# zafarrafii/Zaf-Python

Hardware: AMD Instinct MI355X
Metric: audio Msamples/sec (STFT win=2048 hop=1024) (higher is better)
Workload: dtype f32

## Files before the change

### zaf-python_amd/csrc/zafx_stft.hip

```cpp
#include <algorithm>
#include <type_traits>

#include "zafx_fft.hpp"
#include "zafx_units.hpp"
#include "zafx_internal.hpp"

namespace zafx {

template <int SPEC>
__device__ __forceinline__ float2* spec_base(float2* out, long long off) {
    if constexpr (SPEC >= 2) return reinterpret_cast<float2*>(reinterpret_cast<float*>(out) + off);
    else return out + off;
}
template <int SPEC, bool STREAM = false>
__device__ __forceinline__ void put_bin(float2* o, long long idx, float2 v) {
    if constexpr (SPEC >= 2) {
        const float pw = v.x * v.x + v.y * v.y;
        reinterpret_cast<float*>(o)[idx] = SPEC == 2 ? __builtin_amdgcn_sqrtf(pw) : pw;
    } else if constexpr (STREAM) {
        store_stream(o + idx, v);
    } else {
        o[idx] = v;
    }
}

template <int LOG2N, int LOG2E, int FPB>
struct StftCfg {
    using C = FftCfg<LOG2N, LOG2E>;
    static constexpr int NT = FPB * C::P;
    static constexpr bool TW_LDS = (size_t)(FPB * C::PITCH + C::TW) * 8 <= (size_t)kMaxLdsBytes;
    static constexpr size_t SMEM = (size_t)(FPB * C::PITCH + (TW_LDS ? C::TW : 0)) * 8;
};

template <int LOG2N, int LOG2E, int FPB, int LAYOUT, int SPEC>
__global__ __launch_bounds__(FPB * fft_threads(LOG2N, LOG2E)) void k_stft(
    const float* __restrict__ x, const float* __restrict__ win, const float2* __restrict__ twp,
    const float2* __restrict__ tws, float2* __restrict__ out, long long n_samples, int hop, int T, int TP, int tiles) {
    using C = FftCfg<LOG2N, LOG2E>;
    using S = StftCfg<LOG2N, LOG2E, FPB>;
    constexpr int N = C::N, P = C::P, E = C::E, W = 2 * N, NT = S::NT, ROWS = SPEC ? N + 1 : W;
    extern __shared__ __attribute__((aligned(16))) unsigned char smem_raw[];
    float2* frames = reinterpret_cast<float2*>(smem_raw);
    const float2* tw = twp;
    const int tid = threadIdx.x;
    if constexpr (S::TW_LDS) {
        float2* tw_l = frames + FPB * C::PITCH;
        for (int i = tid; i < C::TW; i += NT) tw_l[i] = twp[i];
        tw = tw_l;
        __syncthreads();
    }
    const int slot = tid / P, p = tid % P;
    const int bid = ZAFX_XCD_ORDER ? xcd_order((int)blockIdx.x, (int)gridDim.x) : (int)blockIdx.x;
    const int clip = bid / tiles, tile = bid % tiles;
    const int t0 = tile * FPB;
    const int t = t0 + slot;
    float2* buf = frames + slot * C::PITCH;

    float2 v[E];
    {
        const float* xc = x + (long long)clip * n_samples;
        const long long s0 = (long long)t * hop - N;
        const float2* w2 = reinterpret_cast<const float2*>(win);
        if (t < T && s0 >= 0 && s0 + W <= n_samples && reinterpret_cast<uintptr_t>(xc + s0) % 8 == 0) {
            const float2* x2 = reinterpret_cast<const float2*>(xc + s0);
#pragma unroll
            for (int i = 0; i < E; ++i) {
                const int n = p + i * P;
                const float2 xv = x2[n], wv = w2[n];
                v[i] = make_float2(xv.x * wv.x, xv.y * wv.y);
            }
        } else {
#pragma unroll
            for (int i = 0; i < E; ++i) {
                const int n = p + i * P;
                const long long s = s0 + 2 * n;
                const float2 wv = w2[n];
                const float a = (t < T && s >= 0 && s < n_samples) ? xc[s] : 0.f;
                const float b = (t < T && s + 1 >= 0 && s + 1 < n_samples) ? xc[s + 1] : 0.f;
                v[i] = make_float2(a * wv.x, b * wv.y);
            }
        }
    }
    fft_frame<LOG2N, LOG2E>(v, buf, p, tw);

    if constexpr (LAYOUT == ZAFX_LAYOUT_TF) {
        if (t >= T) return;
        float2* o = spec_base<SPEC>(out, ((long long)clip * T + t) * ROWS);
#pragma unroll
        for (int i = 0; i < E / 2; ++i) {
            const int k = p + i * P;
            if (k == 0) {
                const float2 z0 = buf[0], zc = buf[phys(N / 2)];
                put_bin<SPEC>(o, 0, make_float2(z0.x + z0.y, 0.f));
                put_bin<SPEC>(o, N, make_float2(z0.x - z0.y, 0.f));
                put_bin<SPEC>(o, N / 2, cconj(zc));
                if (SPEC == 0) put_bin<SPEC>(o, N + N / 2, zc);
            } else {
                float2 xk, xn;
                split_pair(buf[phys(k)], buf[phys(N - k)], tws[k], xk, xn);
                put_bin<SPEC>(o, k, xk);
                put_bin<SPEC>(o, N - k, xn);
                if (SPEC == 0) {
                    put_bin<SPEC>(o, W - k, cconj(xk));
                    put_bin<SPEC>(o, N + k, cconj(xn));
                }
            }
        }
    } else {
        if constexpr (NT > 64) __syncthreads();
        const int tt = tid % FPB, kq = tid / FPB;
        if (t0 + tt >= T) return;
        const float2* fb = frames + tt * C::PITCH;
        float2* o = spec_base<SPEC>(out, (long long)clip * ROWS * TP + (t0 + tt));
        for (int k = kq; k < N / 2; k += P) {
            if (k == 0) {
                const float2 z0 = fb[0], zc = fb[phys(N / 2)];
                put_bin<SPEC>(o, 0, make_float2(z0.x + z0.y, 0.f));
                put_bin<SPEC>(o, (long long)N * TP, make_float2(z0.x - z0.y, 0.f));
                put_bin<SPEC>(o, (long long)(N / 2) * TP, cconj(zc));
                if (SPEC == 0) put_bin<SPEC>(o, (long long)(N + N / 2) * TP, zc);
            } else {
                float2 xk, xn;
                split_pair(fb[phys(k)], fb[phys(N - k)], tws[k], xk, xn);
                put_bin<SPEC>(o, (long long)k * TP, xk);
                put_bin<SPEC>(o, (long long)(N - k) * TP, xn);
                if (SPEC == 0) {
                    put_bin<SPEC>(o, (long long)(W - k) * TP, cconj(xk));
                    put_bin<SPEC>(o, (long long)(N + k) * TP, cconj(xn));
                }
            }
        }
    }
}

ZAFX_PROF_ARRAY(g_prof_stft)
ZAFX_PROF_TAIL_PTR(g_stft_tail)
constexpr int kFatWaves = 8;
constexpr int kFatFrames = 16;

template <int LOG2N, int LOG2E, int FPB_ = kFatFrames>
struct FatCfg {
    using C = FftCfg<LOG2N, LOG2E>;
    static_assert(C::P == 64 || C::P == 32, "a frame is owned by one wavefront, or by half of one (32 points per thread)");
    static constexpr int N = C::N;
    static constexpr int FPB = FPB_;
    static constexpr bool WIN_LDS = FPB_ == kFatFrames;
    static constexpr int PITCH = ((N + (N >> C::PS) + 31) / 32) * 32 + 32 / FPB_;
    static constexpr int NT = kFatWaves * 64;
    static constexpr int FPW = FPB_ * C::P / NT;
    static constexpr size_t SMEM = (size_t)(FPB_ * PITCH + C::TW + (WIN_LDS ? N : 0) + N / 2 + 1) * 8;
};

template <int PCM>
struct PcmPoint {
    using T = std::conditional_t<PCM == 1, float, float2>;
    static __device__ __forceinline__ float2 get(T v) {
        if constexpr (PCM == 1) {
            const int d = __builtin_bit_cast(int, v);
            return make_float2((float)(short)(d & 0xffff), (float)(d >> 16));
        } else if constexpr (PCM == 2) {
            const int a = __builtin_bit_cast(int, v.x), b = __builtin_bit_cast(int, v.y);
            return make_float2((float)((int)(short)(a & 0xffff) + (a >> 16)), (float)((int)(short)(b & 0xffff) + (b >> 16)));
        } else {
            return v;
        }
    }
    static constexpr float scale() { return PCM == 1 ? 1.f / 32768.f : PCM == 2 ? 1.f / 65536.f : 1.f; }
};

#ifndef ZAFX_STFT_FAT_OPAQUE
#define ZAFX_STFT_FAT_OPAQUE(log2n, spec) ((log2n) == 8 || ((log2n) == 9 && (spec) <= 1))
#endif
template <int LOG2N, int LOG2E, bool ALIGNED, int SPEC, int FPB_ = kFatFrames, int PCM = 0, bool RAGGED = false, bool DYN = false>
__global__ __launch_bounds__(kFatWaves * 64) void k_stft_ft16(
    const float* __restrict__ x, const float* __restrict__ win, const float2* __restrict__ twp,
    const float2* __restrict__ tws, float2* __restrict__ out, SamplesArg<RAGGED> n_samples, int hop, int T, int TP, int tiles,
    TilesArg<DYN> tiles_arg) {
    static_assert(!RAGGED || (FPB_ == kFatFrames && (PCM == 0 || LOG2N == 10)), "ragged batches: 16-frame tiles; int16 samples at W = 2048");
    static_assert(!DYN || FPB_ == kFatFrames, "claimed tiles: 16-frame tiles");
    const int& total_tiles = tiles_total<DYN>(tiles_arg);
#define CLIP_N rg_pick<RAGGED>(rc.n_samples, n_samples)
#define CLIP_T rg_pick<RAGGED>(rc.T, T)
#define CLIP_TP rg_pick<RAGGED>(rc.TP, TP)
    using C = FftCfg<LOG2N, LOG2E>;
    using F = FatCfg<LOG2N, LOG2E, FPB_>;
    constexpr int N = C::N, P = C::P, E = C::E, W = 2 * N, NT = F::NT, FPB = F::FPB, FPW = F::FPW, PITCH = F::PITCH;
    static_assert(FPW >= 1, "every group of P lanes transforms at least one frame per tile");
    constexpr int ROWS = SPEC ? N + 1 : W;
    extern __shared__ __attribute__((aligned(16))) unsigned char smem_raw[];
    float2* frames = reinterpret_cast<float2*>(smem_raw);
    float2* tw_l = frames + FPB * PITCH;
    float2* win_s = tw_l + C::TW;
    float2* tws_l = win_s + (F::WIN_LDS ? N : 0);
    const float2* win_l = F::WIN_LDS ? win_s : reinterpret_cast<const float2*>(win);
    const int tid = threadIdx.x;
    [[maybe_unused]] int* const slot = reinterpret_cast<int*>(tws_l + N / 2 + 1);
    [[maybe_unused]] const int home = (int)blockIdx.x & (kClaimQueues - 1);
    [[maybe_unused]] int cq = home, ticket = 0;
    [[maybe_unused]] bool live = false;
    [[maybe_unused]] auto draw = [&](int q) { return atomicAdd(tiles_claim<DYN>(tiles_arg) + q * kClaimStride, 1); };
    if constexpr (DYN) {
        if (tid == 0) {
            const int c0 = claim_finish(cq, home, total_tiles, draw(cq), draw);
            const int c1 = c0 >= 0 ? claim_finish(cq, home, total_tiles, draw(cq), draw) : -1;
            slot[2] = c0;
            slot[1] = c1;
            live = c1 >= 0;
        }
    }
    for (int i = tid; i < C::TW; i += NT) tw_l[i] = twp[i];
    static_assert(PCM == 0 || F::WIN_LDS, "int16 input: the staged window carries the scale");
    using PP = PcmPoint<PCM>;
    if constexpr (F::WIN_LDS)
        for (int i = tid; i < N; i += NT) {
            const float2 wv = reinterpret_cast<const float2*>(win)[i];
            win_s[i] = make_float2(wv.x * PP::scale(), wv.y * PP::scale());
        }
    for (int i = tid; i <= N / 2; i += NT) tws_l[i] = tws[i];
    __syncthreads();
    const int wave = tid / P, p_lane = tid % P, p = p_lane;
    const int tt = tid % FPB, kq = tid / FPB;
    const float2* fb = frames + tt * PITCH;
    const bool lines_whole = (RAGGED || TP % 16 == 0) && reinterpret_cast<uintptr_t>(out) % 128 == 0;

    typename PP::T xr[FPW][E];
    [[maybe_unused]] const bool xcd = ZAFX_XCD_ORDER && gridDim.x % 8 == 0;
    auto prefetch = [&](int tlv) {
        if (DYN ? tlv < 0 : tlv >= total_tiles) return;
        const int tl = DYN ? tlv : xcd ? xcd_order(tlv, total_tiles) : tlv;
        int p = p_lane;
        if constexpr (E >= 32 || ZAFX_STFT_FAT_OPAQUE(LOG2N, SPEC)) asm volatile("" : "+v"(p));
        [[maybe_unused]] RgClip rc;
        if constexpr (RAGGED) rc = rg_clip(n_samples, tiles, tl);
        const int clip = RAGGED ? 0 : tl / tiles, tile = RAGGED ? tl - rc.first_tile : tl % tiles;
        const float* xc = x + (RAGGED ? rc.in_off : (long long)clip * CLIP_N);
        const long long first = (long long)tile * FPB * hop - N;
        const long long last = first + (long long)(FPB - 1) * hop + W;
        if constexpr (PCM == 1) {
            const short* xs = reinterpret_cast<const short*>(x) + (RAGGED ? rc.in_off : (long long)clip * CLIP_N);
            if (ALIGNED && first >= 0 && last <= CLIP_N && tile * FPB + FPB <= CLIP_T) {
                const short* src = xs + first + (long long)(wave * FPW) * hop + 2 * p;
#pragma unroll
                for (int f = 0; f < FPW; ++f) {
#pragma unroll
                    for (int i = 0; i < E; ++i) xr[f][i] = *reinterpret_cast<const float*>(src + (long long)f * hop + 2 * i * P);
                }
            } else {
#pragma unroll
                for (int f = 0; f < FPW; ++f) {
                    const int t = tile * FPB + wave * FPW + f;
                    const long long s0 = (long long)t * hop - N;
#pragma unroll
                    for (int i = 0; i < E; ++i) {
                        const long long s = s0 + 2 * (p + i * P);
                        const unsigned lo = (t < CLIP_T && s >= 0 && s < CLIP_N) ? (unsigned short)xs[s] : 0u;
                        const unsigned hi = (t < CLIP_T && s + 1 >= 0 && s + 1 < CLIP_N) ? (unsigned short)xs[s + 1] : 0u;
                        xr[f][i] = __builtin_bit_cast(float, lo | hi << 16);
                    }
                }
            }
        } else if (ALIGNED && first >= 0 && last <= CLIP_N && tile * FPB + FPB <= CLIP_T) {
            const float* src = xc + first + (long long)(wave * FPW) * hop + 2 * p;
#pragma unroll
            for (int f = 0; f < FPW; ++f) {
#pragma unroll
                for (int i = 0; i < E; ++i) xr[f][i] = *reinterpret_cast<const float2*>(src + (long long)f * hop + 2 * i * P);
            }
        } else {
#pragma unroll
            for (int f = 0; f < FPW; ++f) {
                const int t = tile * FPB + wave * FPW + f;
                const long long s0 = (long long)t * hop - N;
#pragma unroll
                for (int i = 0; i < E; ++i) {
                    const long long s = s0 + 2 * (p + i * P);
                    xr[f][i].x = (t < CLIP_T && s >= 0 && s < CLIP_N) ? xc[s] : 0.f;
                    xr[f][i].y = (t < CLIP_T && s + 1 >= 0 && s + 1 < CLIP_N) ? xc[s + 1] : 0.f;
                }
            }
        }
    };
    int tlv = blockIdx.x;
    if constexpr (DYN) tlv = __builtin_amdgcn_readfirstlane(slot[2]);
    [[maybe_unused]] int par = 0;
    prefetch(tlv);
    PROF_INIT(g_prof_stft);
    PROF_TAIL_INIT();
    while (DYN ? tlv >= 0 : tlv < total_tiles) {
        const int tl = DYN ? tlv : xcd ? xcd_order(tlv, total_tiles) : tlv;
        [[maybe_unused]] RgClip rc;
        if constexpr (RAGGED) rc = rg_clip(n_samples, tiles, tl);
        const int clip = RAGGED ? 0 : tl / tiles, tile = RAGGED ? tl - rc.first_tile : tl % tiles;
        const int t0 = tile * FPB;
        PROF_MARK(0);
        int po = p;
        if constexpr (E >= 32 || ZAFX_STFT_FAT_OPAQUE(LOG2N, SPEC)) asm volatile("" : "+v"(po));
#pragma unroll
        for (int f = 0; f < FPW; ++f) {
            float2 v[E];
            if constexpr (DYN) {
                if (f == FPW - 1) {
#pragma unroll
                    for (int i = 0; i < E; ++i) {
                        if constexpr (PCM == 1) asm volatile("" : "+v"(xr[f][i])::"memory");
                        else asm volatile("" : "+v"(xr[f][i].x), "+v"(xr[f][i].y)::"memory");
                    }
                    if (tid == 0 && live) ticket = draw(cq);
                }
            }
#pragma unroll
            for (int i = 0; i < E; ++i) {
                const float2 wv = win_l[po + i * P], xv = PP::get(xr[f][i]);
                v[i] = make_float2(xv.x * wv.x, xv.y * wv.y);
            }
            fft_frame<LOG2N, LOG2E>(v, frames + (wave * FPW + f) * PITCH, po, tw_l);
        }
#ifndef ZAFX_STFT_EARLY
#define ZAFX_STFT_EARLY 1
#endif
        if constexpr (DYN) {
            if (tid == 0) {
                const int c = live ? claim_finish(cq, home, total_tiles, ticket, draw) : -1;
                slot[par] = c;
                live = c >= 0;
            }
        }
        int nxt = tlv + gridDim.x;
        if constexpr (DYN) nxt = __builtin_amdgcn_readfirstlane(slot[par ^ 1]);
        if (ZAFX_STFT_EARLY) prefetch(nxt);
        PROF_MARK(1);
        lds_barrier();
        PROF_MARK(2);
        if (!ZAFX_STFT_EARLY) prefetch(nxt);
        PROF_TAIL_FIRST();
        PROF_MARK(3);
        if (t0 + tt < CLIP_T) {
            float2* o = spec_base<SPEC>(out, (RAGGED ? rc.out_off : (long long)clip * ROWS * TP) + (t0 + tt));
            int kqo = kq;
            if constexpr (E >= 32 || ZAFX_STFT_FAT_OPAQUE(LOG2N, SPEC)) asm volatile("" : "+v"(kqo));
            auto store_tile = [&](auto stream) {
                constexpr bool ST = decltype(stream)::value;
                constexpr int ITER = (N / 2) / (NT / FPB);
#ifndef ZAFX_STFT_ROWROT_EXPR
#define ZAFX_STFT_ROWROT_EXPR (((int)blockIdx.x & 7) * 2 + ((int)blockIdx.x >> 3))
#endif
                static_assert((N / 2) % (NT / FPB) == 0, "the row sweep is a whole number of iterations");
                const int rot = ST ? ZAFX_STFT_ROWROT_EXPR : 0;
                for (int it = 0; it < ITER; ++it) {
                    const int k = kqo + ((it + rot) % ITER) * (NT / FPB);
                    if (k == 0) {
                        const float2 z0 = fb[0], zc = fb[phys_t<C::PS>(N / 2)];
                        put_bin<SPEC, ST>(o, 0, make_float2(z0.x + z0.y, 0.f));
                        put_bin<SPEC, ST>(o, (long long)N * CLIP_TP, make_float2(z0.x - z0.y, 0.f));
                        put_bin<SPEC, ST>(o, (long long)(N / 2) * CLIP_TP, cconj(zc));
                        if (SPEC == 0) put_bin<SPEC, ST>(o, (long long)(N + N / 2) * CLIP_TP, zc);
                    } else {
                        float2 xk, xn;
                        split_pair(fb[phys_t<C::PS>(k)], fb[phys_t<C::PS>(N - k)], tws_l[k], xk, xn);
                        put_bin<SPEC, ST>(o, (long long)k * CLIP_TP, xk);
                        if (SPEC == 0) put_bin<SPEC, ST>(o, (long long)(W - k) * CLIP_TP, cconj(xk));
                        put_bin<SPEC, ST>(o, (long long)(N - k) * CLIP_TP, xn);
                        if (SPEC == 0) put_bin<SPEC, ST>(o, (long long)(N + k) * CLIP_TP, cconj(xn));
                    }
                }
            };
#ifndef ZAFX_STFT_NO_NT
            if (SPEC < 2 && lines_whole && FPB == 16) store_tile(std::true_type{});
            else
#endif
                store_tile(std::false_type{});
        }
        PROF_MARK(4);
        lds_barrier();
        tlv = nxt;
        par ^= 1;
        PROF_TAIL_TILE();
    }
    PROF_TAIL_END(g_stft_tail);
    if constexpr (DYN) {
        if (tid == 0) {
            int* const cnt = tiles_claim<DYN>(tiles_arg);
            if (atomicAdd(cnt + kClaimQueues * kClaimStride, 1) == (int)gridDim.x - 1)
                for (int i = 0; i <= kClaimQueues; ++i) atomicExch(cnt + i * kClaimStride, 0);
        }
    }
}
#undef CLIP_N
#undef CLIP_T
#undef CLIP_TP

template <int LOG2N, int LOG2E, bool ALIGNED, int SPEC, int PCM = 0>
__global__ __launch_bounds__(kFatWaves * 64) void k_stft_ft16c(
    const float* __restrict__ x, const float* __restrict__ win, const float2* __restrict__ twp,
    const float2* __restrict__ tws, float2* __restrict__ out, long long n_samples, int hop, int T, int TP, int tiles,
    int segs, int seg_tiles, int units) {
    static_assert(SPEC < 2, "complex spectra only (the real kinds write 64-byte runs)");
    using C = FftCfg<LOG2N, LOG2E>;
    using F = FatCfg<LOG2N, LOG2E>;
    constexpr int N = C::N, P = C::P, E = C::E, W = 2 * N, NT = F::NT, FPB = kFatFrames, FPW = F::FPW, PITCH = F::PITCH;
    constexpr int ROWS = SPEC ? N + 1 : W;
    constexpr int ITER = (N / 2) / (NT / FPB);
    static_assert((N / 2) % (NT / FPB) == 0 && ITER >= 1, "the row sweep is a whole number of iterations");
    extern __shared__ __attribute__((aligned(16))) unsigned char smem_raw[];
    float2* frames = reinterpret_cast<float2*>(smem_raw);
    float2* tw_l = frames + FPB * PITCH;
    float2* win_l = tw_l + C::TW;
    float2* tws_l = win_l + N;
    const int tid = threadIdx.x;
    for (int i = tid; i < C::TW; i += NT) tw_l[i] = twp[i];
    using PP = PcmPoint<PCM>;
    static_assert(PCM == 0 || ALIGNED, "int16 input: the buffer-load form");
    for (int i = tid; i < N; i += NT) {
        const float2 wv = reinterpret_cast<const float2*>(win)[i];
        win_l[i] = make_float2(wv.x * PP::scale(), wv.y * PP::scale());
    }
    for (int i = tid; i <= N / 2; i += NT) tws_l[i] = tws[i];
    __syncthreads();
    const int wave = tid / P, p_lane = tid % P;
    const int tt = tid % FPB, kq = tid / FPB;
    const float2* fb = frames + tt * PITCH;
    const bool xcd = ZAFX_XCD_ORDER && gridDim.x % 8 == 0;
    const int b0 = (int)((reinterpret_cast<uintptr_t>(out) >> 3) & 15);

    typename PP::T xr[FPW][E];
    auto prefetch = [&](int clip, int tile) {
        const float* xc = x + (long long)clip * n_samples;
        if constexpr (ALIGNED) {
            if constexpr (PCM == 1) {
                const __amdgpu_buffer_rsrc_t rs = make_rsrc(reinterpret_cast<const short*>(x) + (long long)clip * n_samples, (unsigned)(n_samples * 2));
#pragma unroll
                for (int f = 0; f < FPW; ++f) {
                    const int s0 = (tile * FPB + wave * FPW + f) * hop - N;
                    const int vo = (s0 + 2 * p_lane) * 2;
#pragma unroll
                    for (int i = 0; i < E; ++i) xr[f][i] = buf_load_f32(rs, vo + i * P * 4);
                }
            } else {
            const __amdgpu_buffer_rsrc_t rs = make_rsrc(xc, (unsigned)(n_samples * 4));
#pragma unroll
            for (int f = 0; f < FPW; ++f) {
                const int s0 = (tile * FPB + wave * FPW + f) * hop - N;
                const int vo = (s0 + 2 * p_lane) * 4;
#pragma unroll
                for (int i = 0; i < E; ++i) xr[f][i] = buf_load_f32x2(rs, vo + i * P * 8);
            }
            }
        } else if constexpr (PCM != 1) {
#pragma unroll
            for (int f = 0; f < FPW; ++f) {
                const int t = tile * FPB + wave * FPW + f;
                const long long s0 = (long long)t * hop - N;
#pragma unroll
                for (int i = 0; i < E; ++i) {
                    const long long s = s0 + 2 * (p_lane + i * P);
                    xr[f][i].x = (t < T && s >= 0 && s < n_samples) ? xc[s] : 0.f;
                    xr[f][i].y = (t < T && s + 1 >= 0 && s + 1 < n_samples) ? xc[s + 1] : 0.f;
                }
            }
        }
    };
    auto unit_of = [&](int v, int& clip, int& j, int& j1) {
        const int u = xcd ? xcd_order(v, units) : v;
        clip = u / segs;
        j = (u % segs) * seg_tiles;
        j1 = min(j + seg_tiles, tiles);
    };
    int v = blockIdx.x;
    if (v >= units) return;
    int clip, j, j1;
    unit_of(v, clip, j, j1);
    prefetch(clip, j);
    float2 ck[ITER], cn[ITER];
#pragma unroll
    for (int it = 0; it < ITER; ++it) ck[it] = cn[it] = make_float2(0.f, 0.f);
    bool have_prev = false;
    for (;;) {
        int po = p_lane;
        asm volatile("" : "+v"(po));
#pragma unroll
        for (int f = 1; f < FPW; ++f) {
            float2* park = frames + (wave * FPW + f) * PITCH;
#pragma unroll
            for (int i = 0; i < E; ++i) {
                const float2 wv = win_l[po + i * P], xv = PP::get(xr[f][i]);
                park[po + i * P] = make_float2(xv.x * wv.x, xv.y * wv.y);
            }
        }
#pragma unroll
        for (int f = 0; f < FPW; ++f) {
            float2 vv[E];
            float2* buf = frames + (wave * FPW + f) * PITCH;
            if (f == 0) {
#pragma unroll
                for (int i = 0; i < E; ++i) {
                    const float2 wv = win_l[po + i * P], xv = PP::get(xr[0][i]);
                    vv[i] = make_float2(xv.x * wv.x, xv.y * wv.y);
                }
            } else {
                frame_sync<P>();
#pragma unroll
                for (int i = 0; i < E; ++i) vv[i] = buf[po + i * P];
                frame_sync<P>();
            }
            fft_frame<LOG2N, LOG2E>(vv, buf, po, tw_l);
            __builtin_amdgcn_sched_barrier(0);
        }
        int nclip = clip, nj = j + 1, nj1 = j1, nv = v;
        bool more = true;
        if (nj >= j1) {
            nv = v + gridDim.x;
            if (nv < units) unit_of(nv, nclip, nj, nj1);
            else more = false;
        }
        if (more) prefetch(nclip, nj);
        lds_barrier();
        {
            const int t0 = j * FPB;
            const bool last = j + 1 >= j1, cur_ok = t0 + tt < T;
            float2* o = out + (long long)clip * ROWS * TP + (t0 + tt);
            const int c0 = (int)(((long long)clip * ROWS) & 15), tp = TP & 15;
            int kqo = kq;
            asm volatile("" : "+v"(kqo));
            auto sweep = [&](auto stream) {
                constexpr bool ST = decltype(stream)::value;
                auto emit = [&](int r, float2 cur, float2 prev) {
                    const int a = (b0 + (c0 + r) * tp) & 15;
                    const bool from_prev = tt >= 16 - a;
                    const float2 val = from_prev ? prev : cur;
                    float2* dst = o + (long long)r * TP;
                    if (from_prev ? have_prev : cur_ok) {
                        if constexpr (ST) store_stream(dst + (from_prev ? -16 : 0), val);
                        else dst[from_prev ? -16 : 0] = val;
                    }
                    if (last && from_prev && cur_ok) *dst = cur;
                };
#pragma unroll
                for (int it = 0; it < ITER; ++it) {
                    const int k = kqo + it * (NT / FPB);
                    float2 xk, xn;
                    if (it == 0 && k == 0) {
                        const float2 z0 = fb[0], zc = fb[phys_t<C::PS>(N / 2)];
                        xk = cconj(zc);
                        xn = make_float2(z0.x + z0.y, z0.x - z0.y);
                        emit(N / 2, xk, ck[0]);
                        if (SPEC == 0) emit(N + N / 2, cconj(xk), cconj(ck[0]));
                        emit(0, make_float2(xn.x, 0.f), make_float2(cn[0].x, 0.f));
                        emit(N, make_float2(xn.y, 0.f), make_float2(cn[0].y, 0.f));
                    } else {
                        split_pair(fb[phys_t<C::PS>(k)], fb[phys_t<C::PS>(N - k)], tws_l[k], xk, xn);
                        emit(k, xk, ck[it]);
                        if (SPEC == 0) emit(W - k, cconj(xk), cconj(ck[it]));
                        emit(N - k, xn, cn[it]);
                        if (SPEC == 0) emit(N + k, cconj(xn), cconj(cn[it]));
                    }
                    ck[it] = xk;
                    cn[it] = xn;
                    __builtin_amdgcn_sched_barrier(0);
                }
            };
            if (have_prev) sweep(std::true_type{});
            else sweep(std::false_type{});
        }
        lds_barrier();
        if (!more) break;
        have_prev = nj != 0 && nv == v;
        clip = nclip, j = nj, j1 = nj1, v = nv;
    }
}

struct BandCfg {
    using C = FftCfg<10, 4>;
    static constexpr int N = 1024, M = 2048, W = 4096, FPB = kFatFrames, NT = kFatWaves * 64, FPW = 2;
    static constexpr int PITCH = FatCfg<10, 4>::PITCH;
    static constexpr size_t SMEM = (size_t)(FPB * PITCH + C::TW + M / 2 + 1) * 8;
};
static_assert(BandCfg::SMEM <= (size_t)kMaxLdsBytes, "k_stft_ft16b: tile + tables exceed LDS");

template <bool ALIGNED, int SPEC>
__global__ __launch_bounds__(kFatWaves * 64) void k_stft_ft16b(
    const float* __restrict__ x, const float* __restrict__ win, const float2* __restrict__ twp,
    const float2* __restrict__ tws, float2* __restrict__ out, long long n_samples, int hop, int T, int TP, int tiles,
    int total_tiles) {
    using B = BandCfg;
    using C = B::C;
    constexpr int N = B::N, M = B::M, W = B::W, P = 64, E = 16, NT = B::NT, FPB = B::FPB, FPW = B::FPW, PITCH = B::PITCH;
    constexpr int ROWS = SPEC ? M + 1 : W;
    extern __shared__ __attribute__((aligned(16))) unsigned char smem_raw[];
    float2* frames = reinterpret_cast<float2*>(smem_raw);
    float2* tw_l = frames + FPB * PITCH;
    float2* tws_l = tw_l + C::TW;
    const int tid = threadIdx.x;
    for (int i = tid; i < C::TW; i += NT) tw_l[i] = twp[i];
    for (int i = tid; i <= M / 2; i += NT) tws_l[i] = tws[i];
    __syncthreads();
    const int wave = tid / P, p_lane = tid % P;
    const int tt = tid % FPB, kq = tid / FPB;
    const float2* fb = frames + tt * PITCH;
    const bool lines_whole = TP % 16 == 0 && reinterpret_cast<uintptr_t>(out) % 128 == 0;
    const bool xcd = ZAFX_XCD_ORDER && gridDim.x % 8 == 0;
    const float2 wp = tws_l[2 * p_lane];

    float2 xr[FPW][2 * E];
    auto prefetch = [&](int tlv) {
        if (tlv >= total_tiles) return;
        const int tl = xcd ? xcd_order(tlv, total_tiles) : tlv;
        const int clip = tl / tiles, tile = tl % tiles;
        const float* xc = x + (long long)clip * n_samples;
        const __amdgpu_buffer_rsrc_t rs = make_rsrc(xc, (unsigned)(n_samples * 4));
#pragma unroll
        for (int f = 0; f < FPW; ++f) {
            const int s0 = (tile * FPB + wave * FPW + f) * hop - M;
            const int vo = (s0 + 2 * p_lane) * 4;
            int vo1 = vo + 4;
            if constexpr (!ALIGNED) asm volatile("" : "+v"(vo1));
#pragma unroll
            for (int j = 0; j < 2 * E; ++j) {
                if constexpr (ALIGNED) {
                    xr[f][j] = buf_load_f32x2(rs, vo + j * P * 8);
                } else {
                    xr[f][j].x = buf_load_f32(rs, vo + j * P * 8);
                    xr[f][j].y = buf_load_f32(rs, vo1 + j * P * 8);
                }
            }
        }
    };
    auto store_band = [&](auto band, auto stream, float2* o) {
        constexpr int S = decltype(band)::value;
        constexpr bool ST = decltype(stream)::value;
        constexpr int ITER = (N / 2) / (NT / FPB);
        static_assert((N / 2) % (NT / FPB) == 0, "the row sweep is a whole number of iterations");
        int kqo = kq;
        asm volatile("" : "+v"(kqo));
        const int rot = ST ? ZAFX_STFT_ROWROT_EXPR : 0;
        for (int it = 0; it < ITER; ++it) {
            const int q = kqo + ((it + rot) % ITER) * (NT / FPB);
            if (S == 0 && q == 0) {
                const float2 z0 = fb[0], zc = fb[phys_t<C::PS>(N / 2)];
                put_bin<SPEC, ST>(o, 0, make_float2(z0.x + z0.y, 0.f));
                put_bin<SPEC, ST>(o, (long long)M * TP, make_float2(z0.x - z0.y, 0.f));
                put_bin<SPEC, ST>(o, (long long)(M / 2) * TP, cconj(zc));
                if (SPEC == 0) put_bin<SPEC, ST>(o, (long long)(M + M / 2) * TP, zc);
            } else {
                const int k = 2 * q + S;
                float2 xk, xn;
                split_pair(fb[phys_t<C::PS>(q)], fb[phys_t<C::PS>(N - S - q)], tws_l[k], xk, xn);
                put_bin<SPEC, ST>(o, (long long)k * TP, xk);
                if (SPEC == 0) put_bin<SPEC, ST>(o, (long long)(W - k) * TP, cconj(xk));
                put_bin<SPEC, ST>(o, (long long)(M - k) * TP, xn);
                if (SPEC == 0) put_bin<SPEC, ST>(o, (long long)(M + k) * TP, cconj(xn));
            }
        }
    };
    int tlv = blockIdx.x;
    prefetch(tlv);
    for (; tlv < total_tiles; tlv += gridDim.x) {
        const int tl = xcd ? xcd_order(tlv, total_tiles) : tlv;
        const int clip = tl / tiles, tile = tl % tiles;
        const int t0 = tile * FPB;
        int po = p_lane;
        asm volatile("" : "+v"(po));
        {
            const float2* w2 = reinterpret_cast<const float2*>(win) + po;
            const float c32[16] = {1.f, 0.98078528040323044913f, 0.92387953251128675613f, 0.83146961230254523708f, 0.70710678118654752440f,
                                   0.55557023301960222474f, 0.38268343236508977173f, 0.19509032201612826785f, 0.f,
                                   -0.19509032201612826785f, -0.38268343236508977173f, -0.55557023301960222474f, -0.70710678118654752440f,
                                   -0.83146961230254523708f, -0.92387953251128675613f, -0.98078528040323044913f};
            const float s32[16] = {0.f, 0.19509032201612826785f, 0.38268343236508977173f, 0.55557023301960222474f, 0.70710678118654752440f,
                                   0.83146961230254523708f, 0.92387953251128675613f, 0.98078528040323044913f, 1.f,
                                   0.98078528040323044913f, 0.92387953251128675613f, 0.83146961230254523708f, 0.70710678118654752440f,
                                   0.55557023301960222474f, 0.38268343236508977173f, 0.19509032201612826785f};
            float2 wv[2 * E];
#pragma unroll
            for (int j = 0; j < 2 * E; ++j) wv[j] = w2[j * P];
#pragma unroll
            for (int f = 0; f < FPW; ++f) {
#pragma unroll
                for (int i = 0; i < E; ++i) {
                    const float2 a = make_float2(xr[f][i].x * wv[i].x, xr[f][i].y * wv[i].y);
                    const float2 b = make_float2(xr[f][i + E].x * wv[i + E].x, xr[f][i + E].y * wv[i + E].y);
// ... 2439 lines not shown
```

Measured before the change: 281,000.

## Hoist stream choice out of tile loop and make store sweep branch-uniform

The streaming-versus-plain store decision moves outside the persistent tile loop, so each variant is a whole loop specialisation. For DYN non-ragged kernels the streaming path is always taken, with no lines_whole check. The row sweep is fully unrolled, and out-of-range frame lanes are clamped to frame 0 rather than skipped, so every lane issues the same store sequence without divergence. A samples_in asm barrier pins prefetched registers at the end of each tile to control scheduling. The risks are more code size and register pressure, redundant stores from clamped lanes, and streaming stores on DYN paths with unaligned output.

```diff
diff --git a/zaf-python_amd/csrc/zafx_stft.hip b/zaf-python_amd/csrc/zafx_stft.hip
--- a/zaf-python_amd/csrc/zafx_stft.hip
+++ b/zaf-python_amd/csrc/zafx_stft.hip
@@ -149,6 +149,8 @@
     static constexpr int NT = kFatWaves * 64;
     static constexpr int FPW = FPB_ * C::P / NT;
     static constexpr size_t SMEM = (size_t)(FPB_ * PITCH + C::TW + (WIN_LDS ? N : 0) + N / 2 + 1) * 8;
+    template <int SPEC>
+    static constexpr int kSweepStores = (N / 2) / (NT / FPB_) * (SPEC == 0 ? 4 : 2);
 };
 
 template <int PCM>
@@ -220,12 +222,11 @@
     __syncthreads();
     const int wave = tid / P, p_lane = tid % P, p = p_lane;
     const int tt = tid % FPB, kq = tid / FPB;
-    const float2* fb = frames + tt * PITCH;
-    const bool lines_whole = (RAGGED || TP % 16 == 0) && reinterpret_cast<uintptr_t>(out) % 128 == 0;
+    [[maybe_unused]] const bool lines_whole = (RAGGED || TP % 16 == 0) && reinterpret_cast<uintptr_t>(out) % 128 == 0;
 
     typename PP::T xr[FPW][E];
     [[maybe_unused]] const bool xcd = ZAFX_XCD_ORDER && gridDim.x % 8 == 0;
-    auto prefetch = [&](int tlv) {
+    auto prefetch = [&](int tlv) __attribute__((always_inline)) {
         if (DYN ? tlv < 0 : tlv >= total_tiles) return;
         const int tl = DYN ? tlv : xcd ? xcd_order(tlv, total_tiles) : tlv;
         int p = p_lane;
@@ -280,101 +281,149 @@
             }
         }
     };
+    auto samples_in = [&]() __attribute__((always_inline)) {
+#pragma unroll
+        for (int f = 0; f < FPW; ++f) {
+#pragma unroll
+            for (int i = 0; i < E; ++i) {
+                if constexpr (PCM == 1) asm volatile("" : "+v"(xr[f][i]));
+                else asm volatile("" : "+v"(xr[f][i].x), "+v"(xr[f][i].y));
+            }
+        }
+    };
     int tlv = blockIdx.x;
     if constexpr (DYN) tlv = __builtin_amdgcn_readfirstlane(slot[2]);
     [[maybe_unused]] int par = 0;
     prefetch(tlv);
+    samples_in();
     PROF_INIT(g_prof_stft);
     PROF_TAIL_INIT();
-    while (DYN ? tlv >= 0 : tlv < total_tiles) {
-        const int tl = DYN ? tlv : xcd ? xcd_order(tlv, total_tiles) : tlv;
-        [[maybe_unused]] RgClip rc;
-        if constexpr (RAGGED) rc = rg_clip(n_samples, tiles, tl);
-        const int clip = RAGGED ? 0 : tl / tiles, tile = RAGGED ? tl - rc.first_tile : tl % tiles;
-        const int t0 = tile * FPB;
-        PROF_MARK(0);
-        int po = p;
-        if constexpr (E >= 32 || ZAFX_STFT_FAT_OPAQUE(LOG2N, SPEC)) asm volatile("" : "+v"(po));
-#pragma unroll
-        for (int f = 0; f < FPW; ++f) {
-            float2 v[E];
-            if constexpr (DYN) {
-                if (f == FPW - 1) {
-#pragma unroll
-                    for (int i = 0; i < E; ++i) {
-                        if constexpr (PCM == 1) asm volatile("" : "+v"(xr[f][i])::"memory");
-                        else asm volatile("" : "+v"(xr[f][i].x), "+v"(xr[f][i].y)::"memory");
+    auto run_tiles = [&](auto stream) __attribute__((always_inline)) {
+        constexpr bool ST = decltype(stream)::value;
+        while (DYN ? tlv >= 0 : tlv < total_tiles) {
+            const int tl = DYN ? tlv : xcd ? xcd_order(tlv, total_tiles) : tlv;
+            [[maybe_unused]] RgClip rc;
+            if constexpr (RAGGED) rc = rg_clip(n_samples, tiles, tl);
+            const int clip = RAGGED ? 0 : tl / tiles, tile = RAGGED ? tl - rc.first_tile : tl % tiles;
+            const int t0 = tile * FPB;
+            PROF_MARK(0);
+#ifdef ZAFX_PROF
+            samples_in();
+            PROF_MARK(5);
+#endif
+            int po = p;
+            if constexpr (E >= 32 || ZAFX_STFT_FAT_OPAQUE(LOG2N, SPEC)) asm volatile("" : "+v"(po));
+#pragma unroll
+            for (int f = 0; f < FPW; ++f) {
+                float2 v[E];
+                if constexpr (DYN) {
+                    if (f == FPW - 1) {
+#pragma unroll
+                        for (int i = 0; i < E; ++i) {
+                            if constexpr (PCM == 1) asm volatile("" : "+v"(xr[f][i])::"memory");
+                            else asm volatile("" : "+v"(xr[f][i].x), "+v"(xr[f][i].y)::"memory");
+                        }
+                        if (tid == 0 && live) ticket = draw(cq);
                     }
-                    if (tid == 0 && live) ticket = draw(cq);
-                }
-            }
-#pragma unroll
-            for (int i = 0; i < E; ++i) {
-                const float2 wv = win_l[po + i * P], xv = PP::get(xr[f][i]);
-                v[i] = make_float2(xv.x * wv.x, xv.y * wv.y);
-            }
-            fft_frame<LOG2N, LOG2E>(v, frames + (wave * FPW + f) * PITCH, po, tw_l);
-        }
+                }
+#pragma unroll
+                for (int i = 0; i < E; ++i) {
+                    const float2 wv = win_l[po + i * P], xv = PP::get(xr[f][i]);
+                    v[i] = make_float2(xv.x * wv.x, xv.y * wv.y);
+                }
+                fft_frame<LOG2N, LOG2E>(v, frames + (wave * FPW + f) * PITCH, po, tw_l);
+            }
 #ifndef ZAFX_STFT_EARLY
 #define ZAFX_STFT_EARLY 1
 #endif
-        if constexpr (DYN) {
-            if (tid == 0) {
-                const int c = live ? claim_finish(cq, home, total_tiles, ticket, draw) : -1;
-                slot[par] = c;
-                live = c >= 0;
-            }
-        }
-        int nxt = tlv + gridDim.x;
-        if constexpr (DYN) nxt = __builtin_amdgcn_readfirstlane(slot[par ^ 1]);
-        if (ZAFX_STFT_EARLY) prefetch(nxt);
-        PROF_MARK(1);
-        lds_barrier();
-        PROF_MARK(2);
-        if (!ZAFX_STFT_EARLY) prefetch(nxt);
-        PROF_TAIL_FIRST();
-        PROF_MARK(3);
-        if (t0 + tt < CLIP_T) {
-            float2* o = spec_base<SPEC>(out, (RAGGED ? rc.out_off : (long long)clip * ROWS * TP) + (t0 + tt));
-            int kqo = kq;
-            if constexpr (E >= 32 || ZAFX_STFT_FAT_OPAQUE(LOG2N, SPEC)) asm volatile("" : "+v"(kqo));
-            auto store_tile = [&](auto stream) {
-                constexpr bool ST = decltype(stream)::value;
-                constexpr int ITER = (N / 2) / (NT / FPB);
+            if constexpr (DYN) {
+                if (tid == 0) {
+                    const int c = live ? claim_finish(cq, home, total_tiles, ticket, draw) : -1;
+                    slot[par] = c;
+                    live = c >= 0;
+                }
+            }
+            int nxt = tlv + gridDim.x;
+            if constexpr (DYN) nxt = __builtin_amdgcn_readfirstlane(slot[par ^ 1]);
+            if (ZAFX_STFT_EARLY) prefetch(nxt);
+            PROF_MARK(1);
+            lds_barrier();
+            PROF_MARK(2);
+            if (!ZAFX_STFT_EARLY) prefetch(nxt);
+            PROF_TAIL_FIRST();
+            PROF_MARK(3);
+            {
+                const int tte = t0 + tt < CLIP_T ? tt : 0;
+                const float2* fb = frames + tte * PITCH;
+                float2* o = spec_base<SPEC>(out, (RAGGED ? rc.out_off : (long long)clip * ROWS * TP) + (t0 + tte));
+                int kqo = kq;
+                if constexpr (E >= 32 || ZAFX_STFT_FAT_OPAQUE(LOG2N, SPEC)) asm volatile("" : "+v"(kqo));
+                {
+                    constexpr int ITER = (N / 2) / (NT / FPB);
 #ifndef ZAFX_STFT_ROWROT_EXPR
 #define ZAFX_STFT_ROWROT_EXPR (((int)blockIdx.x & 7) * 2 + ((int)blockIdx.x >> 3))
 #endif
-                static_assert((N / 2) % (NT / FPB) == 0, "the row sweep is a whole number of iterations");
-                const int rot = ST ? ZAFX_STFT_ROWROT_EXPR : 0;
-                for (int it = 0; it < ITER; ++it) {
-                    const int k = kqo + ((it + rot) % ITER) * (NT / FPB);
-                    if (k == 0) {
-                        const float2 z0 = fb[0], zc = fb[phys_t<C::PS>(N / 2)];
-                        put_bin<SPEC, ST>(o, 0, make_float2(z0.x + z0.y, 0.f));
-                        put_bin<SPEC, ST>(o, (long long)N * CLIP_TP, make_float2(z0.x - z0.y, 0.f));
-                        put_bin<SPEC, ST>(o, (long long)(N / 2) * CLIP_TP, cconj(zc));
-                        if (SPEC == 0) put_bin<SPEC, ST>(o, (long long)(N + N / 2) * CLIP_TP, zc);
-                    } else {
-                        float2 xk, xn;
-                        split_pair(fb[phys_t<C::PS>(k)], fb[phys_t<C::PS>(N - k)], tws_l[k], xk, xn);
-                        put_bin<SPEC, ST>(o, (long long)k * CLIP_TP, xk);
-                        if (SPEC == 0) put_bin<SPEC, ST>(o, (long long)(W - k) * CLIP_TP, cconj(xk));
-                        put_bin<SPEC, ST>(o, (long long)(N - k) * CLIP_TP, xn);
-                        if (SPEC == 0) put_bin<SPEC, ST>(o, (long long)(N + k) * CLIP_TP, cconj(xn));
+                    static_assert((N / 2) % (NT / FPB) == 0, "the row sweep is a whole number of iterations");
+                    int rot = ST ? ZAFX_STFT_ROWROT_EXPR : 0;
+                    if constexpr (ST) asm volatile("" : "+s"(rot));
+                    static_assert(F::template kSweepStores<SPEC> == ITER * (SPEC == 0 ? 4 : 2), "the stores of a sweep that every lane issues");
+                    static_assert(F::template kSweepStores<SPEC> >= 4 && F::template kSweepStores<SPEC> % ITER == 0, "two iterations at the least (W = 256), the same stores in each");
+#pragma unroll
+                    for (int it = 0; it < ITER; ++it) {
+                        const int k = kqo + ((it + rot) % ITER) * (NT / FPB);
+                        long long r0, r1;
+                        [[maybe_unused]] long long r2 = 0, r3 = 0;
+                        float2 a0, a1;
+                        [[maybe_unused]] float2 a2 = {}, a3 = {};
+                        if (k == 0) {
+                            const float2 z0 = fb[0], zc = fb[phys_t<C::PS>(N / 2)];
+                            r0 = 0, a0 = make_float2(z0.x + z0.y, 0.f);
+                            r1 = N, a1 = make_float2(z0.x - z0.y, 0.f);
+                            r2 = N / 2, a2 = cconj(zc);
+                            r3 = N + N / 2, a3 = zc;
+                        } else {
+                            float2 xk, xn;
+                            split_pair(fb[phys_t<C::PS>(k)], fb[phys_t<C::PS>(N - k)], tws_l[k], xk, xn);
+                            r0 = k, a0 = xk;
+                            if (SPEC == 0) {
+                                r1 = W - k, a1 = cconj(xk);
+                                r2 = N - k, a2 = xn;
+                                r3 = N + k, a3 = cconj(xn);
+                            } else {
+                                r1 = N - k, a1 = xn;
+                            }
+                        }
+                        put_bin<SPEC, ST>(o, r0 * CLIP_TP, a0);
+                        put_bin<SPEC, ST>(o, r1 * CLIP_TP, a1);
+                        if constexpr (SPEC == 0) {
+                            put_bin<SPEC, ST>(o, r2 * CLIP_TP, a2);
+                            put_bin<SPEC, ST>(o, r3 * CLIP_TP, a3);
+                        } else {
+                            if (k == 0) put_bin<SPEC, ST>(o, r2 * CLIP_TP, a2);
+                        }
                     }
                 }
-            };
+            }
+            samples_in();
+            PROF_MARK(4);
+            lds_barrier();
+            tlv = nxt;
+            par ^= 1;
+            PROF_TAIL_TILE();
+        }
+    };
 #ifndef ZAFX_STFT_NO_NT
-            if (SPEC < 2 && lines_whole && FPB == 16) store_tile(std::true_type{});
-            else
+    constexpr bool CAN_STREAM = SPEC < 2 && FPB == 16;
+#else
+    constexpr bool CAN_STREAM = false;
 #endif
-                store_tile(std::false_type{});
-        }
-        PROF_MARK(4);
-        lds_barrier();
-        tlv = nxt;
-        par ^= 1;
-        PROF_TAIL_TILE();
+    if constexpr (CAN_STREAM && DYN && !RAGGED) {
+        run_tiles(std::true_type{});
+    } else if constexpr (CAN_STREAM) {
+        if (lines_whole) run_tiles(std::true_type{});
+        else run_tiles(std::false_type{});
+    } else {
+        run_tiles(std::false_type{});
     }
     PROF_TAIL_END(g_stft_tail);
     if constexpr (DYN) {
```

Result: no change. 279,300 (median of 2 runs) (-0.6%).
